# google/deepconsensus

Measured on AMD Instinct MI355X. Metric: zmw_per_sec, higher is better.
Workload: dtype bf16; 1 GPU; global_batch=16384, seq_len=100, windows_per_zmw=150, parallelism=dp1, native_kernels=True, hipgraph=True

## Files before the change

deepconsensus_amd/models/runner.py:

```python
from __future__ import annotations

import copy
import math
from typing import List, Optional, Tuple

import torch

from deepconsensus_amd import ops as dc_ops
from deepconsensus_amd.calibration.calibration import (
    parse_calibration_string,
)
from deepconsensus_amd.models.config import Params
from deepconsensus_amd.models.model import (
    EncoderOnlyLearnedValuesTransformer,
    get_model,
)
from deepconsensus_amd.utils import constants
from deepconsensus_amd.utils import trace


def build_gather_tables(model: EncoderOnlyLearnedValuesTransformer):
    (bi, pwi, ipi, sti, ci, bqi, sni) = model.indices

    def scaled(emb):
        t = emb.table.detach().float() * math.sqrt(emb.width)
        t = t.clone()
        t[0].zero_()
        return t.to(torch.bfloat16)

    tables = {
        "bases": scaled(model.bases_embedding),
        "pw": scaled(model.pw_embedding),
        "ip": scaled(model.ip_embedding),
        "strand": scaled(model.strand_embedding),
        "sn": scaled(model.sn_embedding),
    }
    if model.use_ccs_bq:
        tables["ccs_bq"] = scaled(model.ccs_bq_embedding)

    order = ["bases", "pw", "ip", "strand", "sn"]
    if model.use_ccs_bq:
        order.append("ccs_bq")
    flat_parts, table_base = [], {}
    off = 0
    for name in order:
        t = tables[name]
        table_base[name] = off
        flat = t.reshape(-1)
        pad = (-flat.numel()) % 8
        if pad:
            flat = torch.cat([flat, flat.new_zeros(pad)])
        flat_parts.append(flat)
        off += flat.numel()
    table_flat = torch.cat(flat_parts).contiguous()

    plan: List[Tuple[str, int]] = []
    plan += [("bases", 0)] * (bi[1] - bi[0])
    plan += [("pw", 0)] * (pwi[1] - pwi[0])
    plan += [("ip", 0)] * (ipi[1] - ipi[0])
    plan += [("strand", 0)] * (sti[1] - sti[0])
    plan += [("bases", 0)] * (ci[1] - ci[0])
    if model.use_ccs_bq:
        plan += [("ccs_bq", 1)]
    plan += [("sn", 0)] * (sni[1] - sni[0])

    row_shift = torch.tensor([s for _, s in plan], dtype=torch.int32)
    row_vocab = torch.tensor(
        [tables[n].shape[0] for n, _ in plan], dtype=torch.int32
    )

    cols: List[Tuple[int, int, int]] = []
    for r, (name, _) in enumerate(plan):
        w = tables[name].shape[1]
        base = table_base[name]
        for j in range(w):
            cols.append((r, base, w))
    concat = len(cols)
    assert concat % 8 == 0, f"concat width {concat} not 8-aligned"
    nchunk = concat // 8
    chunk_cnt = torch.zeros(nchunk, dtype=torch.int32)
    chunk_entries = torch.zeros(nchunk * 4, 4, dtype=torch.int32)
    for c in range(nchunk):
        entries = []
        j = c * 8
        while j < (c + 1) * 8:
            r, base, w = cols[j]
            entries.append((r, base, w))
            j += w
        assert len(entries) <= 4, "chunk spans >4 table rows"
        if len(entries) == 1:
            assert entries[0][2] == 8, (
                f"chunk {c}: single entry must be width 8, got "
                f"{entries[0][2]} (row layout misaligned)"
            )
        else:
            assert all(w == 2 for _, _, w in entries), (
                f"chunk {c}: multi-entry chunk must be all width-2 "
                f"entries, got {[w for _, _, w in entries]}"
            )
        chunk_cnt[c] = len(entries)
        for k, (r, base, w) in enumerate(entries):
            chunk_entries[c * 4 + k] = torch.tensor([r, base, w, 0])
    return table_flat, row_shift, row_vocab, chunk_cnt, chunk_entries.reshape(-1)


class InferenceRunner:

    def __init__(
        self,
        params: Params,
        model: Optional[torch.nn.Module] = None,
        device: Optional[str] = None,
        calibration: str = "skip",
        max_qual: int = constants.MAX_QUAL,
    ):
        self.params = params
        if device is None:
            device = "cuda" if torch.cuda.is_available() else "cpu"
        self.device = torch.device(device)
        self.calib = parse_calibration_string(calibration)
        self.max_qual = max_qual
        if model is None:
            model = get_model(params)
        model.eval()
        self.model = model

        self.native = (
            self.device.type == "cuda"
            and isinstance(model, EncoderOnlyLearnedValuesTransformer)
            and model.condense
        )
        if self.device.type == "cuda":
            self.ext = dc_ops.get_ext(required=self.native)
        else:
            self.ext = None

        self.model = model.to(self.device)
        if self.native:
            self._prepare_native(model)

    def _prepare_native(self, model) -> None:
        dev, bf16 = self.device, torch.bfloat16
        tf, rs, rv, cc, ce = build_gather_tables(model)
        self.table_flat = tf.to(dev)
        self.row_shift = rs.to(dev)
        self.row_vocab = rv.to(dev)
        self.chunk_cnt = cc.to(dev)
        self.chunk_entries = ce.to(dev)
        self.win = model.params.get("attn_win_size")
        self.num_heads = model.params["num_heads"]
        self.cond_wt = (
            model.condenser.weight.detach().t().contiguous().to(bf16).to(dev)
        )
        self.pos = (
            model.pos_encoding.to(bf16).to(dev)
            if model.add_pos_encoding
            else None
        )
        import os as _os

        self.cond_img = None
        self.pos_f32 = None
        cw = model.condenser.weight.detach()
        if cw.shape[1] == 560 and _os.environ.get("DC_FUSED_CONDENSE") != "0":
            npad = -(-cw.shape[0] // 64) * 64
            img = torch.zeros(npad, 568, dtype=bf16)
            img[: cw.shape[0], :560] = cw.to(bf16)
            self.cond_img = img.contiguous().to(dev)
            if model.add_pos_encoding:
                self.pos_f32 = (
                    model.pos_encoding.detach().float().contiguous().to(dev)
                )
        self.rezero_fast = all(
            l.attn_wrap.rezero and l.ffn_wrap.rezero for l in model.layers
        ) and self.win is not None
        if self.rezero_fast:
            self.layer_w = []
            for l in model.layers:
                wq = l.attn.q_proj.weight.detach()
                wk = l.attn.k_proj.weight.detach()
                wv = l.attn.v_proj.weight.detach()
                wqkv_t = (
                    torch.cat([wq, wk, wv], 0).t().contiguous().to(bf16).to(dev)
                )
                self.layer_w.append(
                    dict(
                        wqkv_t=wqkv_t,
                        wout_t=l.attn.out_proj.weight.detach()
                        .t().contiguous().to(bf16).to(dev),
                        w1_t=l.ffn.filter_layer.weight.detach()
                        .t().contiguous().to(bf16).to(dev),
                        b1=l.ffn.filter_layer.bias.detach().to(bf16).to(dev),
                        w2_t=l.ffn.output_layer.weight.detach()
                        .t().contiguous().to(bf16).to(dev),
                        b2=l.ffn.output_layer.bias.detach().to(bf16).to(dev),
                        alpha_attn=float(l.attn_wrap.alpha.detach()),
                        alpha_ffn=float(l.ffn_wrap.alpha.detach()),
                    )
                )
            for lw in self.layer_w:
                lw["wout_t_a"] = lw["wout_t"] * lw["alpha_attn"]
                lw["w2_t_a"] = lw["w2_t"] * lw["alpha_ffn"]
                lw["b2_a"] = lw["b2"] * lw["alpha_ffn"]
            import os as _os

            self.ffn_fused_ok = (
                model.params["hidden_size"] == 280
                and model.params["filter_size"] == 2048
                and _os.environ.get("DC_FUSED_FFN") != "0"
            )
            self.ffn_v2 = _os.environ.get("DC_FFN_V2", "1") != "0"
            self.ffn_v3 = _os.environ.get("DC_FFN_V3", "1") != "0"

            if self.ffn_fused_ok:
                for i, l in enumerate(model.layers):
                    lw = self.layer_w[i]
                    wq = l.attn.q_proj.weight.detach().float()
                    wk = l.attn.k_proj.weight.detach().float()
                    wv = l.attn.v_proj.weight.detach().float()
                    wqkv = torch.cat([wq, wk, wv], 0)
                    wqkv_pad = torch.zeros(896, 296)
                    wqkv_pad[:840, :280] = wqkv
                    lw["wqkv_pad"] = wqkv_pad.to(bf16).contiguous().to(dev)
                    wo = l.attn.out_proj.weight.detach().float()
                    wout_pad = torch.zeros(320, 296)
                    wout_pad[:280, :280] = wo
                    lw["wout_pad"] = wout_pad.to(bf16).contiguous().to(dev)
                    w1 = l.ffn.filter_layer.weight.detach().float()
                    w1p = torch.zeros(2048, 288)
                    w1p[:, :280] = w1
                    lw["w1_pad"] = w1p.to(bf16).contiguous().to(dev)
                    lw["b1_f32"] = (
                        l.ffn.filter_layer.bias.detach().float().to(dev)
                    )
                    w2 = l.ffn.output_layer.weight.detach().float()
                    w2p = torch.zeros(320, 2048)
                    w2p[:280] = w2
                    lw["w2_pad"] = w2p.to(bf16).contiguous().to(dev)
                    b2p = torch.zeros(320)
                    b2p[:280] = l.ffn.output_layer.bias.detach().float()
                    lw["b2_f32"] = b2p.to(dev)
                    w1v2 = torch.zeros(2048, 296)
                    w1v2[:, :280] = w1
                    w1v2[:, 287] = l.ffn.filter_layer.bias.detach().float()
                    lw["w1_v2"] = w1v2.to(bf16).contiguous().to(dev)
            self._addmm_act = hasattr(torch, "_addmm_activation")
            if self._addmm_act:
                try:
                    torch._addmm_activation(
                        torch.zeros(4, device=dev, dtype=bf16),
                        torch.zeros(2, 4, device=dev, dtype=bf16),
                        torch.zeros(4, 4, device=dev, dtype=bf16),
                    )
                except Exception:
                    self._addmm_act = False
        else:
            layers = copy.deepcopy(model.layers).to(bf16)
            for m in layers.modules():
                if isinstance(m, torch.nn.LayerNorm):
                    m.float()
            self.layers_bf16 = layers.to(dev)
        self.ln_gamma = model.output_norm.weight.detach().float().to(dev)
        self.ln_beta = model.output_norm.bias.detach().float().to(dev)
        self.w_head = model.fc1.weight.detach().float().contiguous().to(dev)
        self.b_head = model.fc1.bias.detach().float().to(dev)

    def _attn(self, qkv: torch.Tensor) -> torch.Tensor:
        b, l, w = qkv.shape
        d = w // (3 * self.num_heads)
        if d == 140 and 32 <= l <= 104 and 1 <= self.win <= 12:
            return self.ext.banded_attn_mfma(
                qkv, self.num_heads, self.win, d ** -0.5
            )
        return self.ext.banded_attn(qkv, self.num_heads, self.win)

    @torch.no_grad()
    def encode_native(self, rows: torch.Tensor) -> torch.Tensor:
        with trace.range("K2_embed_gather"):
            emb = self.ext.embed_gather(
                rows.contiguous(), self.table_flat, self.row_shift,
                self.row_vocab, self.chunk_cnt, self.chunk_entries,
            )
        b, l, _ = emb.shape
        if self.cond_img is not None:
            with trace.range("K3_condenser"):
                h = self.cond_wt.shape[1]
                pos = (
                    self.pos_f32
                    if self.pos_f32 is not None
                    else emb.new_empty(0, dtype=torch.float32)
                )
                x = self.ext.fused_condense(
                    emb.reshape(b * l, -1), self.cond_img, pos, h, l
                )
            x = x.view(b, l, -1)
        else:
            with trace.range("K3_condenser"):
                x = emb.reshape(b * l, -1) @ self.cond_wt
            x = x.view(b, l, -1)
            if self.pos is not None:
                x = x + self.pos[:l]
        if self.rezero_fast:
            h = x.shape[-1]
            flat = x.reshape(b * l, h)
            empty = flat.new_empty(0)
            for lw in self.layer_w:
                with trace.range("K5_qkv_proj"):
                    if self.ffn_fused_ok:
                        qkv = self.ext.fused_linear(
                            flat, lw["wqkv_pad"], empty, empty, 840,
                            False, 0.0
                        ).view(b, l, -1)
                    else:
                        qkv = (flat @ lw["wqkv_t"]).view(b, l, -1)
                with trace.range("K6_banded_attn"):
                    a = self._attn(qkv)
                if self.ffn_fused_ok:
                    with trace.range("K7_out_proj"):
                        flat = self.ext.fused_linear(
                            a.view(b * l, h), lw["wout_pad"], empty, flat,
                            280, False, lw["alpha_attn"],
                        )
                    with trace.range("K9_fused_ffn"):
                        if self.ffn_v3:
                            flat = self.ext.fused_ffn_v3(
                                flat, lw["w1_v2"], lw["w2_pad"],
                                lw["b2_f32"], lw["alpha_ffn"],
                            )
                        elif self.ffn_v2:
                            flat = self.ext.fused_ffn_v2(
                                flat, lw["w1_v2"], lw["w2_pad"],
                                lw["b2_f32"], lw["alpha_ffn"],
                            )
                        else:
                            flat = self.ext.fused_ffn(
                                flat, lw["w1_pad"], lw["b1_f32"],
                                lw["w2_pad"], lw["b2_f32"],
                                lw["alpha_ffn"],
                            )
                    continue
                flat = torch.addmm(flat, a.view(b * l, h), lw["wout_t_a"])
                if self._addmm_act:
                    ff = torch._addmm_activation(lw["b1"], flat, lw["w1_t"])
                    flat = torch.addmm(flat, ff, lw["w2_t_a"]).add_(lw["b2_a"])
                else:
                    ff = torch.addmm(lw["b1"], flat, lw["w1_t"]).relu_()
                    flat = torch.addmm(flat, ff, lw["w2_t_a"]).add_(lw["b2_a"])
            x = flat.view(b, l, h)
        else:
            for layer in self.layers_bf16:
                x, _ = layer(x, training=False)
        return x

    @torch.no_grad()
    def forward_windows_graphed(self, host_rows: torch.Tensor):
        if not self.native:
            return self.forward_windows(host_rows)
        shape = tuple(host_rows.shape)
        if getattr(self, "_graph_shape", None) != shape:
            try:
                g_in = torch.empty(
                    shape, dtype=host_rows.dtype, device=self.device
                )
                side = torch.cuda.Stream()
                side.wait_stream(torch.cuda.current_stream())
                with torch.cuda.stream(side):
                    for _ in range(2):
                        self.forward_windows(g_in)
                torch.cuda.current_stream().wait_stream(side)
                torch.cuda.synchronize()
                graph = torch.cuda.CUDAGraph()
                with torch.cuda.graph(graph):
                    g_bases, g_quals = self.forward_windows(g_in)
                torch.cuda.synchronize()
                self._graph = graph
                self._graph_in = g_in
                self._graph_out = (g_bases, g_quals)
                self._graph_shape = shape
            except Exception:
                self._graph_shape = None
                self._graph = None
                return self.forward_windows(host_rows)
        self._graph_in.copy_(host_rows, non_blocking=True)
        self._graph.replay()
        return self._graph_out

    @torch.no_grad()
    def forward_windows(
        self, rows: torch.Tensor, want_probs: bool = False
    ):
        rows = rows.to(self.device, non_blocking=True)
        if self.native:
            x = self.encode_native(rows)
            with trace.range("K10_K12_ln_head_qv"):
                out = self.ext.fused_ln_head_qv(
                x.reshape(-1, x.shape[-1]),
                self.ln_gamma,
                self.ln_beta,
                self.w_head,
                self.b_head,
                float(self.calib.threshold) if self.calib.enabled else -1.0,
                float(self.calib.w) if self.calib.enabled else 1.0,
                float(self.calib.b) if self.calib.enabled else 0.0,
                float(self.max_qual),
                want_probs,
            )
            b, l = rows.shape[0], rows.shape[2]
            bases = out[0].view(b, l)
            quals = out[1].view(b, l)
            if want_probs:
                return bases, quals, out[2].view(b, l, 5)
            return bases, quals
        probs = self.model(rows)
        return self.probs_to_calls(probs, want_probs)

    def probs_to_calls(self, probs: torch.Tensor, want_probs: bool = False):
        pmax, bases = probs.max(dim=-1)
        ep = (1.0 - pmax).clamp_min(1e-12)
        q = -10.0 * torch.log10(ep)
        if self.calib.enabled:
            if self.calib.threshold == 0:
                q = q * self.calib.w + self.calib.b
            else:
                mask = q > self.calib.threshold
                q = torch.where(mask, q * self.calib.w + self.calib.b, q)
        q = q.clamp_max(self.max_qual)
        q = torch.round(q).clamp_min(0)
        bases = bases.to(torch.uint8)
        quals = q.to(torch.uint8)
        if want_probs:
            return bases, quals, probs
        return bases, quals
```

deepconsensus_amd/ops/build.py:

```python
from __future__ import annotations

import os
import shutil

_OPS_DIR = os.path.dirname(os.path.abspath(__file__))
_BUILD_DIR = os.path.join(_OPS_DIR, "_build")
_SRCS = [
    os.path.join(_OPS_DIR, "hip", "dc_kernels.hip"),
    os.path.join(_OPS_DIR, "hip", "banded_attn.hip"),
    os.path.join(_OPS_DIR, "hip", "banded_attn_mfma.hip"),
    os.path.join(_OPS_DIR, "hip", "embed_gather.hip"),
    os.path.join(_OPS_DIR, "hip", "fused_ffn.hip"),
    os.path.join(_OPS_DIR, "hip", "alignment_dp.hip"),
    os.path.join(_OPS_DIR, "hip", "fused_linear.hip"),
    os.path.join(_OPS_DIR, "hip", "fused_ffn_glds.hip"),
    os.path.join(_OPS_DIR, "hip", "fused_ffn_v3.hip"),
    os.path.join(_OPS_DIR, "hip", "embed_grad.hip"),
    os.path.join(_OPS_DIR, "hip", "alignment_metric.hip"),
    os.path.join(_OPS_DIR, "hip", "ffn_ablate.hip"),
    os.path.join(_OPS_DIR, "hip", "fused_ffn_v4.hip"),
    os.path.join(_OPS_DIR, "hip", "banded_attn_train.hip"),
    os.path.join(_OPS_DIR, "hip", "banded_attn_bwd_mfma.hip"),
    os.path.join(_OPS_DIR, "hip", "fused_condense.hip"),
    os.path.join(_OPS_DIR, "hip", "ffn_train.hip"),
    os.path.join(_OPS_DIR, "hip", "resid_dropout.hip"),
    os.path.join(_OPS_DIR, "hip", "stitch_compact.hip"),
    os.path.join(_OPS_DIR, "hip", "window_featurize.hip"),
    os.path.join(_OPS_DIR, "hip", "passthrough_fill.hip"),
    os.path.join(_OPS_DIR, "hip", "subread_space.hip"),
]
EXT_NAME = "dc_hip_kernels"


_SPACING_SRC = os.path.join(
    os.path.dirname(_OPS_DIR), "preprocess", "_spacing_cpp.cpp"
)


def build_spacing(verbose: bool = False):
    os.makedirs(_BUILD_DIR, exist_ok=True)
    from torch.utils.cpp_extension import load

    return load(
        name="_spacing",
        sources=[_SPACING_SRC],
        build_directory=_BUILD_DIR,
        extra_cflags=["-O3"],
        verbose=verbose,
    )


def build(verbose: bool = False):
    os.environ.setdefault("PYTORCH_ROCM_ARCH", "gfx950")
    os.makedirs(_BUILD_DIR, exist_ok=True)
    from torch.utils.cpp_extension import load

    build_spacing(verbose=verbose)
    module = load(
        name=EXT_NAME,
        sources=_SRCS,
        build_directory=_BUILD_DIR,
        extra_cuda_cflags=["-O3", "--offload-arch=gfx950"],
        verbose=verbose,
    )
    return module


def build_asan(verbose: bool = False):
    os.environ["PYTORCH_ROCM_ARCH"] = "gfx950:xnack+"
    build_dir = os.path.join(_OPS_DIR, "_build_asan")
    os.makedirs(build_dir, exist_ok=True)
    from torch.utils.cpp_extension import load

    flags = ["-O2", "-fsanitize=address", "-shared-libsan"]
    module = load(
        name=EXT_NAME + "_asan",
        sources=_SRCS,
        build_directory=build_dir,
        extra_cuda_cflags=flags,
        extra_ldflags=[],
        verbose=verbose,
    )
    return module


def clean():
    if os.path.isdir(_BUILD_DIR):
        shutil.rmtree(_BUILD_DIR)


if __name__ == "__main__":
    build(verbose=True)
    print("built", EXT_NAME, "in", _BUILD_DIR)
```

deepconsensus_amd/ops/hip/dc_kernels.hip:

```cpp

#ifndef DC_SAN_MAIN
#include <torch/extension.h>
#include <ATen/hip/HIPContext.h>
#endif
#include <hip/hip_runtime.h>
#include <hip/hip_bf16.h>

#define DC_CHECK(x, msg) TORCH_CHECK(x, msg)

using bf16 = __hip_bfloat16;

namespace {

template <typename T>
__global__ __launch_bounds__(256) void fused_ln_head_qv_kernel(
    const T* __restrict__ x, const float* __restrict__ gamma,
    const float* __restrict__ beta, const float* __restrict__ w_head,
    const float* __restrict__ b_head, uint8_t* __restrict__ bases_out,
    uint8_t* __restrict__ quals_out, float* __restrict__ probs_out,
    int N, int H, float cal_threshold, float cal_w, float cal_b,
    float max_qual) {
  const int wave_in_block = threadIdx.x >> 6;
  const int lane = threadIdx.x & 63;
  for (int n = blockIdx.x * 4 + wave_in_block; n < N; n += gridDim.x * 4) {
  const T* xi = x + (size_t)n * H;

  float sum = 0.f, sumsq = 0.f;
  float xv[8];
  int nd = 0;
  for (int d = lane; d < H; d += 64, ++nd) {
    float v;
    if constexpr (std::is_same_v<T, bf16>) v = __bfloat162float(xi[d]);
    else v = xi[d];
    xv[nd] = v;
    sum += v;
    sumsq += v * v;
  }
#pragma unroll
  for (int off = 32; off > 0; off >>= 1) {
    sum += __shfl_xor(sum, off, 64);
    sumsq += __shfl_xor(sumsq, off, 64);
  }
  const float mean = sum / H;
  const float var = sumsq / H - mean * mean;
  const float rstd = rsqrtf(var + 1e-6f);

  float logit[5];
#pragma unroll
  for (int k = 0; k < 5; ++k) logit[k] = 0.f;
  nd = 0;
  for (int d = lane; d < H; d += 64, ++nd) {
    const float normed = (xv[nd] - mean) * rstd * gamma[d] + beta[d];
#pragma unroll
    for (int k = 0; k < 5; ++k) logit[k] += normed * w_head[k * H + d];
  }
#pragma unroll
  for (int off = 32; off > 0; off >>= 1) {
#pragma unroll
    for (int k = 0; k < 5; ++k) logit[k] += __shfl_xor(logit[k], off, 64);
  }

  if (lane == 0) {
    float mx = -1e30f;
#pragma unroll
    for (int k = 0; k < 5; ++k) {
      logit[k] += b_head[k];
      mx = fmaxf(mx, logit[k]);
    }
    float denom = 0.f;
    float ex[5];
#pragma unroll
    for (int k = 0; k < 5; ++k) {
      ex[k] = __expf(logit[k] - mx);
      denom += ex[k];
    }
    int arg = 0;
    float pmax = 0.f;
#pragma unroll
    for (int k = 0; k < 5; ++k) {
      const float p = ex[k] / denom;
      if (probs_out != nullptr) probs_out[(size_t)n * 5 + k] = p;
      if (p > pmax) { pmax = p; arg = k; }
    }
    float ep = 1.f - pmax;
    float q = (ep <= 0.f) ? 1e9f : -10.f * log10f(ep);
    if (cal_threshold == 0.f || q > cal_threshold) q = q * cal_w + cal_b;
    q = fminf(q, max_qual);
    q = nearbyintf(q);
    q = fmaxf(q, 0.f);
    bases_out[n] = (uint8_t)arg;
    quals_out[n] = (uint8_t)q;
  }
  }
}

}

#ifndef DC_SAN_MAIN

std::vector<at::Tensor> fused_ln_head_qv(
    at::Tensor x, at::Tensor gamma, at::Tensor beta, at::Tensor w_head,
    at::Tensor b_head, double cal_threshold, double cal_w, double cal_b,
    double max_qual, bool want_probs) {
  DC_CHECK(x.is_cuda() && x.dim() >= 2, "x must be a device matrix");
  auto xc = x.contiguous();
  const int H = xc.size(-1);
  const int N = xc.numel() / H;
  DC_CHECK(H <= 512, "H must be <= 512");
  auto opts = xc.options();
  auto bases = at::empty({N}, opts.dtype(at::kByte));
  auto quals = at::empty({N}, opts.dtype(at::kByte));
  at::Tensor probs;
  float* probs_ptr = nullptr;
  if (want_probs) {
    probs = at::empty({N, 5}, opts.dtype(at::kFloat));
    probs_ptr = probs.data_ptr<float>();
  }
  dim3 grid(std::min((N + 3) / 4, 2048));
  dim3 block(256);
  hipStream_t stream = at::hip::getCurrentHIPStream();
  auto gc = gamma.contiguous(), bc = beta.contiguous();
  auto wc = w_head.contiguous(), bhc = b_head.contiguous();
  if (xc.dtype() == at::kBFloat16) {
    hipLaunchKernelGGL(fused_ln_head_qv_kernel<bf16>, grid, block, 0, stream,
                       reinterpret_cast<bf16*>(xc.data_ptr()),
                       gc.data_ptr<float>(), bc.data_ptr<float>(),
                       wc.data_ptr<float>(), bhc.data_ptr<float>(),
                       bases.data_ptr<uint8_t>(), quals.data_ptr<uint8_t>(),
                       probs_ptr, N, H, (float)cal_threshold, (float)cal_w,
                       (float)cal_b, (float)max_qual);
  } else {
    DC_CHECK(xc.dtype() == at::kFloat, "x must be bf16 or fp32");
    hipLaunchKernelGGL(fused_ln_head_qv_kernel<float>, grid, block, 0, stream,
                       xc.data_ptr<float>(), gc.data_ptr<float>(),
                       bc.data_ptr<float>(), wc.data_ptr<float>(),
                       bhc.data_ptr<float>(), bases.data_ptr<uint8_t>(),
                       quals.data_ptr<uint8_t>(), probs_ptr, N, H,
                       (float)cal_threshold, (float)cal_w, (float)cal_b,
                       (float)max_qual);
  }
  if (want_probs) return {bases, quals, probs};
  return {bases, quals};
}

at::Tensor banded_attn(at::Tensor qkv, int64_t H, int64_t win);
at::Tensor banded_attn_mfma(at::Tensor qkv, int64_t H, int64_t win,
                            double scale);
at::Tensor embed_gather(at::Tensor rows, at::Tensor table_flat,
                        at::Tensor row_shift, at::Tensor row_vocab,
                        at::Tensor chunk_cnt, at::Tensor chunk_entries);
at::Tensor fused_ffn(at::Tensor x, at::Tensor w1, at::Tensor b1,
                     at::Tensor w2, at::Tensor b2, double alpha);
at::Tensor fused_ffn_v2(at::Tensor x, at::Tensor w1, at::Tensor w2,
                        at::Tensor b2, double alpha);
at::Tensor fused_ffn_v3(at::Tensor x, at::Tensor w1, at::Tensor w2,
                        at::Tensor b2, double alpha);
void embed_grad(at::Tensor rows, at::Tensor grad_out, at::Tensor row_shift,
                at::Tensor row_vocab, at::Tensor row_tbase,
                at::Tensor row_width, at::Tensor row_col,
                at::Tensor row_scale, at::Tensor grad_tables);
at::Tensor fused_linear(at::Tensor x, at::Tensor w, at::Tensor bias,
                        at::Tensor resid, int64_t n_out, bool relu,
                        double alpha);
std::vector<at::Tensor> alignment_dp_fwd(at::Tensor subs, at::Tensor ins,
                                         at::Tensor seq_lens, double del_cost,
                                         double reg, int64_t width);
std::vector<at::Tensor> alignment_dp_bwd(at::Tensor grad_out,
                                         at::Tensor weights,
                                         at::Tensor seq_lens, int64_t m,
                                         int64_t n, int64_t width);
std::vector<at::Tensor> alignment_metric_counts(
    at::Tensor yt, at::Tensor yp, at::Tensor yt_len, at::Tensor yp_len,
    double ms, double mp, double go, double ge);
at::Tensor ffn_ablate(at::Tensor x, at::Tensor w1, at::Tensor w2,
                      at::Tensor b2, double alpha, int64_t mode);
at::Tensor fused_ffn_v4(at::Tensor x, at::Tensor w1, at::Tensor w2,
                        at::Tensor b2, double alpha);
std::vector<at::Tensor> banded_attn_train_fwd(
    at::Tensor q, at::Tensor k, at::Tensor v, at::Tensor mask,
    int64_t win, double p_drop);
std::vector<at::Tensor> banded_attn_train_bwd(
    at::Tensor q, at::Tensor k, at::Tensor v, at::Tensor p,
    at::Tensor mask, at::Tensor dout, int64_t win, double p_drop);
std::vector<at::Tensor> banded_attn_mfma_train_fwd(
    at::Tensor qkv, int64_t H, int64_t win, double scale,
    at::Tensor drop_mask, double p_drop);
at::Tensor banded_attn_train_bwd2(
    at::Tensor qkv, at::Tensor p, at::Tensor mask, at::Tensor dout,
    int64_t H, int64_t win, double p_drop);
at::Tensor banded_attn_bwd_mfma(
    at::Tensor qkv, at::Tensor p, at::Tensor mask, at::Tensor dout,
    int64_t H, int64_t win, double p_drop);
at::Tensor fused_condense(at::Tensor x, at::Tensor w, at::Tensor pos,
                          int64_t n_out, int64_t seq_len);
std::vector<at::Tensor> ffn_train_fwd(at::Tensor x, at::Tensor w1,
                                      at::Tensor w2, at::Tensor b2,
                                      double p_drop, int64_t seed);
std::vector<at::Tensor> ffn_train_dgrad(at::Tensor dy, at::Tensor hd,
                                        at::Tensor w2t, at::Tensor w1t,
                                        double p_drop);
std::vector<at::Tensor> ffn_train_dgrad_nomask(at::Tensor dy, at::Tensor hd,
                                               at::Tensor w2t,
                                               at::Tensor w1t,
                                               double p_drop);
at::Tensor resid_drop_fwd(at::Tensor x, at::Tensor y, double alpha,
                          double p_drop, int64_t seed);
std::vector<at::Tensor> resid_drop_bwd(at::Tensor dout, at::Tensor y,
                                       double alpha, double p_drop,
                                       int64_t seed);
std::vector<at::Tensor> stitch_compact(at::Tensor bases, at::Tensor quals,
                                       at::Tensor seg_off,
                                       at::Tensor seg_len);
int64_t stitch_compact_into(at::Tensor bases, at::Tensor quals,
                            at::Tensor seg_off, at::Tensor seg_len,
                            at::Tensor seq_out, at::Tensor qual_out,
                            at::Tensor seg_kept, at::Tensor out_off);
at::Tensor window_featurize(at::Tensor sub, at::Tensor ccs,
                            at::Tensor ccs_bq, at::Tensor zmw_tab,
                            at::Tensor win_tab, int64_t R, int64_t L,
                            int64_t max_passes, bool use_ccs_bq);
void window_featurize_into(at::Tensor sub, at::Tensor ccs,
                           at::Tensor ccs_bq, at::Tensor zmw_tab,
                           at::Tensor win_tab, at::Tensor out,
                           int64_t max_passes, bool use_ccs_bq);
void passthrough_fill_into(at::Tensor ccs, at::Tensor ccs_q,
                           at::Tensor zmw_tab, at::Tensor pt_tab,
                           at::Tensor qual_lut, at::Tensor bases_out,
                           at::Tensor quals_out);
void subread_space_into(at::Tensor src, at::Tensor ins_max,
                        at::Tensor sp_tab, at::Tensor read_tab,
                        at::Tensor zmw_tab, at::Tensor col_ref,
                        at::Tensor sub, at::Tensor ccs, at::Tensor ccs_q,
                        at::Tensor ccs_bq, bool use_ccs_bq);
int64_t subread_space_tile();

PYBIND11_MODULE(TORCH_EXTENSION_NAME, m) {
  m.def("subread_space_into", &subread_space_into,
        "Device subread spacing: unspaced reads + ins_max -> caller-owned "
        "zero-filled sub / ccs / ccs_q / ccs_bq planes");
  m.def("subread_space_tile", &subread_space_tile,
        "Scan tile (elements) of subread_space_into");
  m.def("passthrough_fill_into", &passthrough_fill_into,
        "Device CCS passthrough: skipped windows of the packed planes -> "
        "caller-owned base-id and QV rows of the stitch buffer");
  m.def("window_featurize", &window_featurize,
        "Device window featurization: compact ZMW planes + window table "
        "-> int16 [N, R, L] model input");
  m.def("window_featurize_into", &window_featurize_into,
        "window_featurize into a caller-owned int16 [N, R, L] tensor");
  m.def("stitch_compact", &stitch_compact,
        "Device window stitching: segmented gap compaction -> (seq_out, "
        "qual_out, seg_kept, out_off)");
  m.def("stitch_compact_into", &stitch_compact_into,
        "stitch_compact into caller-owned output buffers; returns "
        "out_off[S]");
  m.def("fused_condense", &fused_condense,
        "Condenser GEMM [M,560]x[560,N] + fused position-encoding add "
        "(K3+K4)");
  m.def("ffn_train_fwd", &ffn_train_fwd,
        "Training FFN forward: relu + hash dropout in-register, returns "
        "(y, hd)");
  m.def("ffn_train_dgrad", &ffn_train_dgrad,
        "Training FFN dgrad: both transposed GEMMs fused, mask from hd>0, "
        "returns (dx, dh_pre)");
  m.def("ffn_train_dgrad_nomask", &ffn_train_dgrad_nomask,
        "Bisection probe: dgrad without the mask (dh == dy@W2^T)");
  m.def("resid_drop_fwd", &resid_drop_fwd,
        "Fused ReZero residual + hash-dropout forward");
  m.def("resid_drop_bwd", &resid_drop_bwd,
        "Fused residual-dropout backward: (dy, dalpha partials)");
  m.def("fused_ln_head_qv", &fused_ln_head_qv,
        "Fused final LayerNorm + head + softmax + QV (K10+K11+K12)");
  m.def("banded_attn", &banded_attn,
        "Banded multi-head self-attention forward (K5-K7 core, generic)");
  m.def("banded_attn_mfma", &banded_attn_mfma,
        "Banded MHA forward on MFMA (D=140, L<=104)");
  m.def("embed_gather", &embed_gather,
        "Subread-stack embedding gather (K2)");
  m.def("fused_ffn", &fused_ffn,
        "Fused FFN + ReZero residual (K8+K9), hidden tensor LDS-resident");
  m.def("fused_ffn_v2", &fused_ffn_v2,
        "Fused FFN v2: glds-pipelined weights, bias folded into W1");
  m.def("fused_ffn_v3", &fused_ffn_v3,
        "Fused FFN v3: 256-row tiles, register-resident h (swapped B1)");
  m.def("embed_grad", &embed_grad,
        "Fused embedding-stack backward (training, all tables, one pass)");
  m.def("fused_linear", &fused_linear,
        "Fused linear projection (K5/K7): act(xW^T+b)[*alpha+x]");
  m.def("alignment_dp_fwd", &alignment_dp_fwd,
        "Alignment-loss wavefront DP forward (K13)");
  m.def("alignment_dp_bwd", &alignment_dp_bwd,
        "Alignment-loss wavefront DP backward (K13 VJP)");
  m.def("alignment_metric_counts", &alignment_metric_counts,
        "Device AlignmentMetric (K14): affine NW + backtrace counts");
  m.def("banded_attn_train_fwd", &banded_attn_train_fwd,
        "Training banded attention forward (saves band softmax P)");
  m.def("banded_attn_mfma_train_fwd", &banded_attn_mfma_train_fwd,
        "MFMA training attention forward (serving kernel + band-P save "
        "+ fused dropout)");
  m.def("banded_attn_bwd_mfma", &banded_attn_bwd_mfma,
        "MFMA training attention backward (band_scores/band_apply "
        "primitives; packed dqkv)");
  m.def("banded_attn_train_bwd2", &banded_attn_train_bwd2,
        "Training attention backward v2 (packed qkv layout, 2 blocks/"
        "CU) -> packed dqkv");
  m.def("banded_attn_train_bwd", &banded_attn_train_bwd,
        "Training banded attention backward (band-local dS -> dq,dk,dv)");
  m.def("fused_ffn_v4", &fused_ffn_v4,
        "Fused FFN v4: B1 on 16x16x32 MFMAs (4 independent chains)");
  m.def("ffn_ablate", &ffn_ablate,
        "fused_ffn_v3 ablation probe (0 full, 1 B1-only, 2 B2-only, "
        "3 loads-only) — perf diagnosis");
}

#endif
```

Before: 2146 ZMWs/sec.

## Add persistent-grid fused FFN v5 with continuous weight streaming across tiles

Adds a new fused FFN kernel that runs the v3 256-row chunk loop in a persistent grid, one block per CU. The next tile's first weight chunk is prefetched during the last chunk of the current tile, so the double-buffered weight stream never drains. The kernel also loads x fragments directly from global memory into registers and uses a 16-byte vectorised residual epilogue staged through LDS. It becomes the default path in the runner. The cost is fewer blocks in flight, one per CU at 512 threads, so latency hiding depends on the pipelining, and there is a risk of load imbalance on the tail tiles.

```diff
diff --git a/deepconsensus_amd/models/runner.py b/deepconsensus_amd/models/runner.py
--- a/deepconsensus_amd/models/runner.py
+++ b/deepconsensus_amd/models/runner.py
@@ -211,6 +211,7 @@
             )
             self.ffn_v2 = _os.environ.get("DC_FFN_V2", "1") != "0"
             self.ffn_v3 = _os.environ.get("DC_FFN_V3", "1") != "0"
+            self.ffn_v5 = _os.environ.get("DC_FFN_V5", "1") != "0"
 
             if self.ffn_fused_ok:
                 for i, l in enumerate(model.layers):
@@ -322,7 +323,12 @@
                             280, False, lw["alpha_attn"],
                         )
                     with trace.range("K9_fused_ffn"):
-                        if self.ffn_v3:
+                        if self.ffn_v5:
+                            flat = self.ext.fused_ffn_v5(
+                                flat, lw["w1_v2"], lw["w2_pad"],
+                                lw["b2_f32"], lw["alpha_ffn"],
+                            )
+                        elif self.ffn_v3:
                             flat = self.ext.fused_ffn_v3(
                                 flat, lw["w1_v2"], lw["w2_pad"],
                                 lw["b2_f32"], lw["alpha_ffn"],
diff --git a/deepconsensus_amd/ops/build.py b/deepconsensus_amd/ops/build.py
--- a/deepconsensus_amd/ops/build.py
+++ b/deepconsensus_amd/ops/build.py
@@ -28,6 +28,7 @@
     os.path.join(_OPS_DIR, "hip", "window_featurize.hip"),
     os.path.join(_OPS_DIR, "hip", "passthrough_fill.hip"),
     os.path.join(_OPS_DIR, "hip", "subread_space.hip"),
+    os.path.join(_OPS_DIR, "hip", "fused_ffn_v5.hip"),
 ]
 EXT_NAME = "dc_hip_kernels"
 
diff --git a/deepconsensus_amd/ops/hip/dc_kernels.hip b/deepconsensus_amd/ops/hip/dc_kernels.hip
--- a/deepconsensus_amd/ops/hip/dc_kernels.hip
+++ b/deepconsensus_amd/ops/hip/dc_kernels.hip
@@ -155,6 +155,8 @@
                         at::Tensor b2, double alpha);
 at::Tensor fused_ffn_v3(at::Tensor x, at::Tensor w1, at::Tensor w2,
                         at::Tensor b2, double alpha);
+at::Tensor fused_ffn_v5(at::Tensor x, at::Tensor w1, at::Tensor w2,
+                        at::Tensor b2, double alpha, int64_t max_blocks);
 void embed_grad(at::Tensor rows, at::Tensor grad_out, at::Tensor row_shift,
                 at::Tensor row_vocab, at::Tensor row_tbase,
                 at::Tensor row_width, at::Tensor row_col,
@@ -283,6 +285,13 @@
         "Fused FFN v2: glds-pipelined weights, bias folded into W1");
   m.def("fused_ffn_v3", &fused_ffn_v3,
         "Fused FFN v3: 256-row tiles, register-resident h (swapped B1)");
+  m.def("fused_ffn_v5", &fused_ffn_v5,
+        "Fused FFN v5: v3 chunk loop in a persistent grid (continuous "
+        "weight stream, direct x fragments, 16-B epilogue); max_blocks "
+        "caps the grid, 0 = one block per CU",
+        pybind11::arg("x"), pybind11::arg("w1"), pybind11::arg("w2"),
+        pybind11::arg("b2"), pybind11::arg("alpha"),
+        pybind11::arg("max_blocks") = 0);
   m.def("embed_grad", &embed_grad,
         "Fused embedding-stack backward (training, all tables, one pass)");
   m.def("fused_linear", &fused_linear,
diff --git a/deepconsensus_amd/ops/hip/fused_ffn_v5.hip b/deepconsensus_amd/ops/hip/fused_ffn_v5.hip
--- /dev/null
+++ b/deepconsensus_amd/ops/hip/fused_ffn_v5.hip
@@ -0,0 +1,325 @@
+
+#ifndef DC_SAN_MAIN
+#include <torch/extension.h>
+#include <ATen/hip/HIPContext.h>
+#endif
+#include <hip/hip_runtime.h>
+#include <hip/hip_bf16.h>
+
+using bf16 = __hip_bfloat16;
+
+namespace {
+
+typedef __bf16 bf16x8 __attribute__((ext_vector_type(8)));
+typedef float f32x16 __attribute__((ext_vector_type(16)));
+typedef float f32x4 __attribute__((ext_vector_type(4)));
+typedef unsigned u32x4 __attribute__((ext_vector_type(4)));
+
+constexpr int BM = 256;
+constexpr int K1 = 280;
+constexpr int K1P = 296;
+constexpr int NC = 64;
+constexpr int NHID = 2048;
+constexpr int NCHUNK = NHID / NC;
+constexpr int W2_STRIDE = 72;
+constexpr int W2_ROWS = 288;
+constexpr int NOUT = 280;
+
+constexpr int W1_ELEMS = NC * K1P;
+constexpr int W2_ELEMS = W2_ROWS * W2_STRIDE;
+constexpr int W1_CHUNKS = W1_ELEMS * 2 / 1024;
+constexpr int W2_GRAN = W2_ROWS * 9;
+constexpr int W2_CHUNKS = (W2_GRAN + 63) / 64;
+
+constexpr int OFF_W1 = 0;
+constexpr int OFF_W2 = 2 * W1_ELEMS;
+constexpr int OFF_SCRATCH = OFF_W2 + 2 * W2_ELEMS;
+constexpr int LDS_ELEMS = OFF_SCRATCH + 1024;
+
+constexpr int EPI_A = W1_ELEMS / 8;
+constexpr int EPI_B = W2_ELEMS / 8;
+constexpr int NQ = NOUT / 8;
+constexpr int EPI_ITERS = (8 * NQ + 63) / 64;
+static_assert(NCHUNK % 2 == 0, "chunk 0 must land in buffer 0 every tile");
+static_assert(EPI_A * 2 >= 4 * NOUT * 4 && EPI_B * 2 >= 4 * NOUT * 4,
+              "a slice holds 4 fp32 rows");
+static_assert((EPI_A * 2) % 16 == 0 && (EPI_B * 2) % 16 == 0,
+              "slices stay 16-B aligned");
+
+__device__ __forceinline__ void glds16(const bf16* gsrc, bf16* ldst) {
+  __builtin_amdgcn_global_load_lds(
+      (const __attribute__((address_space(1))) unsigned*)gsrc,
+      (__attribute__((address_space(3))) unsigned*)ldst, 16, 0, 0);
+}
+
+__device__ __forceinline__ unsigned cvt_pk_bf16(float lo, float hi) {
+  unsigned r;
+  asm volatile("v_cvt_pk_bf16_f32 %0, %1, %2" : "=v"(r) : "v"(lo), "v"(hi));
+  return r;
+}
+
+__device__ __forceinline__ int lane_recompute() {
+  int l;
+  asm volatile(
+      "v_mbcnt_lo_u32_b32 %0, -1, 0\n\t"
+      "v_mbcnt_hi_u32_b32 %0, -1, %0"
+      : "=v"(l));
+  return l;
+}
+
+__device__ __forceinline__ float bf16_lo(unsigned w) {
+  return __uint_as_float(w << 16);
+}
+__device__ __forceinline__ float bf16_hi(unsigned w) {
+  return __uint_as_float(w & 0xffff0000u);
+}
+__device__ __forceinline__ unsigned pack_bf16(float lo, float hi) {
+  return (unsigned)__bfloat16_as_ushort(__float2bfloat16(lo)) |
+         ((unsigned)__bfloat16_as_ushort(__float2bfloat16(hi)) << 16);
+}
+
+__global__ __launch_bounds__(512, 1) void fused_ffn_v5_kernel(
+    const bf16* __restrict__ x, const bf16* __restrict__ w1,
+    const bf16* __restrict__ w2, const float* __restrict__ b2,
+    bf16* __restrict__ out, int M, float alpha, int num_tiles) {
+  __shared__ __attribute__((aligned(16))) bf16 smem[LDS_ELEMS];
+
+  const int wave = __builtin_amdgcn_readfirstlane(threadIdx.x >> 6);
+
+  auto issue_w1 = [&](int chunk, int buf) {
+    const int ln = lane_recompute();
+    const bf16* src = w1 + (size_t)chunk * W1_ELEMS;
+#pragma unroll
+    for (int i = 0; i < 5; ++i) {
+      const int ck = wave + i * 8;
+      if (ck < W1_CHUNKS) {
+        const int dst_off = __builtin_amdgcn_readfirstlane(
+            OFF_W1 + buf * W1_ELEMS + ck * 512);
+        glds16(src + ck * 512 + ln * 8, &smem[dst_off]);
+      }
+    }
+  };
+  auto issue_w2 = [&](int chunk, int buf) {
+    const int ln = lane_recompute();
+#pragma unroll
+    for (int i = 0; i < 6; ++i) {
+      const int ck = wave + i * 8;
+      const int g = ck * 64 + ln;
+      if (g < W2_GRAN) {
+        const int row = g / 9, sub = g % 9;
+        const int k8 = sub == 8 ? 0 : sub;
+        const int dst_off = __builtin_amdgcn_readfirstlane(
+            OFF_W2 + buf * W2_ELEMS + ck * 512);
+        glds16(w2 + (size_t)row * NHID + chunk * NC + 8 * k8,
+               &smem[dst_off]);
+      }
+    }
+  };
+
+  issue_w1(0, 0);
+  issue_w2(0, 0);
+
+  for (int tile = blockIdx.x; tile < num_tiles; tile += gridDim.x) {
+    const int m0 = tile * BM;
+    const bool has_next = tile + (int)gridDim.x < num_tiles;
+
+    bf16x8 af[18];
+    {
+      const int ln = lane_recompute();
+      const int c = ln & 31;
+      const int hi = ln >> 5;
+      const int row = m0 + 32 * wave + c;
+      if (row < M) {
+        const bf16* xr = x + (size_t)row * K1 + 8 * hi;
+#pragma unroll
+        for (int s = 0; s < 17; ++s) {
+          af[s] = *reinterpret_cast<const bf16x8*>(xr + 16 * s);
+        }
+        if (hi == 0) {
+          af[17] = *reinterpret_cast<const bf16x8*>(xr + 16 * 17);
+        } else {
+          af[17] = __builtin_bit_cast(bf16x8, u32x4{0u, 0u, 0u, 0x3f800000u});
+        }
+      } else {
+#pragma unroll
+        for (int s = 0; s < 18; ++s) af[s] = bf16x8{};
+      }
+    }
+
+    asm volatile("s_waitcnt vmcnt(0) lgkmcnt(0)" ::: "memory");
+    __builtin_amdgcn_s_barrier();
+
+    f32x16 oacc[9] = {};
+
+    for (int chunk = 0; chunk < NCHUNK; ++chunk) {
+      const int ln = lane_recompute();
+      const int c = ln & 31;
+      const int hi = ln >> 5;
+      const int buf = chunk & 1;
+      const int nxt = (chunk + 1) & (NCHUNK - 1);
+      if (chunk + 1 < NCHUNK || has_next) {
+        issue_w1(nxt, buf ^ 1);
+        issue_w2(nxt, buf ^ 1);
+      }
+      const bf16* w1buf = &smem[OFF_W1 + buf * W1_ELEMS];
+      const bf16* w2buf = &smem[OFF_W2 + buf * W2_ELEMS];
+
+#pragma unroll
+      for (int t = 0; t < 2; ++t) {
+        f32x16 acc = {};
+        __builtin_amdgcn_s_setprio(1);
+#pragma unroll
+        for (int s = 0; s < 18; ++s) {
+          const bf16x8 wfr = *reinterpret_cast<const bf16x8*>(
+              &w1buf[(32 * t + c) * K1P + 16 * s + 8 * hi]);
+          acc = __builtin_amdgcn_mfma_f32_32x32x16_bf16(wfr, af[s], acc,
+                                                        0, 0, 0);
+        }
+        __builtin_amdgcn_s_setprio(0);
+        float st[16];
+#pragma unroll
+        for (int r = 0; r < 16; ++r) st[r] = acc[r] > 0.f ? acc[r] : 0.f;
+        bf16x8 pa[2];
+#pragma unroll
+        for (int s = 0; s < 2; ++s) {
+          const unsigned x0 = cvt_pk_bf16(st[8 * s + 0], st[8 * s + 1]);
+          const unsigned y0 = cvt_pk_bf16(st[8 * s + 2], st[8 * s + 3]);
+          const unsigned x1 = cvt_pk_bf16(st[8 * s + 4], st[8 * s + 5]);
+          const unsigned y1 = cvt_pk_bf16(st[8 * s + 6], st[8 * s + 7]);
+          const auto rx = __builtin_amdgcn_permlane32_swap(x0, x1, false,
+                                                           false);
+          const auto ry = __builtin_amdgcn_permlane32_swap(y0, y1, false,
+                                                           false);
+          unsigned u[4] = {(unsigned)rx[0], (unsigned)ry[0],
+                           (unsigned)rx[1], (unsigned)ry[1]};
+          pa[s] = *reinterpret_cast<const bf16x8*>(u);
+        }
+        __builtin_amdgcn_s_setprio(1);
+#pragma unroll
+        for (int s = 0; s < 2; ++s) {
+#pragma unroll
+          for (int ct = 0; ct < 9; ++ct) {
+            const int ocol = min(32 * ct + c, NOUT - 1);
+            const bf16x8 wfr = *reinterpret_cast<const bf16x8*>(
+                &w2buf[ocol * W2_STRIDE + 32 * t + 16 * s + 8 * hi]);
+            oacc[ct] = __builtin_amdgcn_mfma_f32_32x32x16_bf16(
+                pa[s], wfr, oacc[ct], 0, 0, 0);
+          }
+        }
+        __builtin_amdgcn_s_setprio(0);
+      }
+
+      asm volatile("s_waitcnt vmcnt(0) lgkmcnt(0)" ::: "memory");
+      __builtin_amdgcn_s_barrier();
+    }
+
+    {
+      const int lne = lane_recompute();
+      const int ce = lne & 31;
+      const int hie = lne >> 5;
+      float* slice_a =
+          reinterpret_cast<float*>(&smem[OFF_W1 + W1_ELEMS + wave * EPI_A]);
+      float* slice_b =
+          reinterpret_cast<float*>(&smem[OFF_W2 + W2_ELEMS + wave * EPI_B]);
+      float* slice_w = hie ? slice_b : slice_a;
+      float bias[9];
+#pragma unroll
+      for (int ct = 0; ct < 9; ++ct) bias[ct] = b2[min(32 * ct + ce, NOUT - 1)];
+      u32x4 rv[4][EPI_ITERS];
+      auto load_resid = [&](int g) {
+#pragma unroll
+        for (int it = 0; it < EPI_ITERS; ++it) {
+          const int idx = min(it * 64 + lne, 8 * NQ - 1);
+          const int row = min(m0 + 32 * wave + 8 * g + idx / NQ, M - 1);
+          rv[g][it] = *reinterpret_cast<const u32x4*>(
+              x + (size_t)row * K1 + 8 * (idx % NQ));
+        }
+      };
+      load_resid(0);
+      load_resid(1);
+      load_resid(2);
+#pragma unroll
+      for (int g = 0; g < 4; ++g) {
+#pragma unroll
+        for (int ct = 0; ct < 9; ++ct) {
+          const int col = 32 * ct + ce;
+          if (col < NOUT) {
+#pragma unroll
+            for (int j = 0; j < 4; ++j) {
+              slice_w[j * NOUT + col] = oacc[ct][4 * g + j] + bias[ct];
+            }
+          }
+        }
+        if (g == 0) load_resid(3);
+        asm volatile("s_waitcnt lgkmcnt(0)" ::: "memory");
+#pragma unroll
+        for (int it = 0; it < EPI_ITERS; ++it) {
+          const int idx = it * 64 + lne;
+          const int rl = idx / NQ, q = idx % NQ;
+          const int row = m0 + 32 * wave + 8 * g + rl;
+          if (idx < 8 * NQ && row < M) {
+            const float* src =
+                (rl < 4 ? slice_a + rl * NOUT : slice_b + (rl - 4) * NOUT) +
+                8 * q;
+            const f32x4 t0 = *reinterpret_cast<const f32x4*>(src);
+            const f32x4 t1 = *reinterpret_cast<const f32x4*>(src + 4);
+            const u32x4 r = rv[g][it];
+            u32x4 ov;
+            ov.x = pack_bf16(bf16_lo(r.x) + alpha * t0.x,
+                             bf16_hi(r.x) + alpha * t0.y);
+            ov.y = pack_bf16(bf16_lo(r.y) + alpha * t0.z,
+                             bf16_hi(r.y) + alpha * t0.w);
+            ov.z = pack_bf16(bf16_lo(r.z) + alpha * t1.x,
+                             bf16_hi(r.z) + alpha * t1.y);
+            ov.w = pack_bf16(bf16_lo(r.w) + alpha * t1.z,
+                             bf16_hi(r.w) + alpha * t1.w);
+            *reinterpret_cast<u32x4*>(out + (size_t)row * K1 + 8 * q) = ov;
+          }
+        }
+        asm volatile("s_waitcnt lgkmcnt(0)" ::: "memory");
+      }
+    }
+  }
+}
+
+}
+
+#ifndef DC_SAN_MAIN
+
+at::Tensor fused_ffn_v5(at::Tensor x, at::Tensor w1, at::Tensor w2,
+                        at::Tensor b2, double alpha, int64_t max_blocks) {
+  TORCH_CHECK(x.is_cuda() && x.dtype() == at::kBFloat16,
+              "x must be bf16 on device");
+  auto xc = x.contiguous();
+  const int K = xc.size(-1);
+  const int M = xc.numel() / K;
+  TORCH_CHECK(K == K1, "fused_ffn_v5 requires width 280");
+  TORCH_CHECK(w1.size(0) == NHID && w1.size(1) == K1P,
+              "w1 must be [2048, 296] with b1 folded into column 287");
+  TORCH_CHECK(w2.size(0) == 320 && w2.size(1) == NHID,
+              "w2 must be padded [320, 2048]");
+  TORCH_CHECK(b2.numel() >= NOUT, "b2 must cover 280 outputs");
+  TORCH_CHECK(max_blocks >= 0, "max_blocks must be >= 0 (0 = one per CU)");
+  auto b2c = b2.contiguous();
+  TORCH_CHECK(b2c.dtype() == at::kFloat, "b2 must be fp32");
+  auto out = at::empty_like(xc);
+  const int num_tiles = (M + BM - 1) / BM;
+  if (num_tiles == 0) return out;
+  const int64_t cap =
+      max_blocks > 0
+          ? max_blocks
+          : at::cuda::getCurrentDeviceProperties()->multiProcessorCount;
+  dim3 grid((unsigned)std::min<int64_t>(num_tiles, cap));
+  dim3 block(512);
+  hipStream_t stream = at::hip::getCurrentHIPStream();
+  hipLaunchKernelGGL(fused_ffn_v5_kernel, grid, block, 0, stream,
+                     reinterpret_cast<bf16*>(xc.data_ptr()),
+                     reinterpret_cast<bf16*>(w1.data_ptr()),
+                     reinterpret_cast<bf16*>(w2.data_ptr()),
+                     b2c.data_ptr<float>(),
+                     reinterpret_cast<bf16*>(out.data_ptr()), M,
+                     (float)alpha, num_tiles);
+  return out;
+}
+
+#endif
```

After: 2466 ZMWs/sec (median of 6 runs). 14.9% higher.
